# GAVLab/feature_extraction

Measured on NVIDIA B200. Metric: scans/sec, higher is better.
Workload: dtype f32

## Files before the change

feature_extraction_b200/csrc/fe_api.cu:

```cuda
#include <algorithm>
#include <cmath>
#include <cstdio>
#include <cstdlib>
#include <cstring>
#include <random>
#include <string>
#include <thread>
#include <vector>

#include "fe_kernels.cuh"

using namespace fe;

#define FE_VERSION "fe_b200 0.1 (sm_100a)"

namespace {

constexpr int GRAPH_MAX_SCANS = 16;
static_assert(GRAPH_MAX_SCANS <= 32, "k_kp_offsets_gather_small gives every scan a warp of one 1024-thread block");
struct GraphKey {
  int nscans, nch, by, k1flags, stride, xo, yo, zo;
  int desc, wantKc, bnd, epoch, lean;
  const void* pts;
  bool operator==(const GraphKey& o) const { return memcmp(this, &o, sizeof(GraphKey)) == 0; }
// ... 413 lines not shown
  CK(cudaFuncSetAttribute(k_ring_runs_wide, cudaFuncAttributeMaxDynamicSharedMemorySize, (int)(NW_RR * sizeof(RunBufT<RW2>))));
  CK(cudaFuncSetAttribute(k_cluster_rings<ECAP_L, NTL, 1, false>, cudaFuncAttributeMaxDynamicSharedMemorySize, (int)kClusterSmemL2));
  CK(cudaFuncSetAttribute(k_merge_keypoints<ECAP_M, NTM, 8, false>, cudaFuncAttributeMaxDynamicSharedMemorySize, (int)kClusterSmemM));
  CK(cudaFuncSetAttribute(k_merge_keypoints<ECAP_L, NT2, 1, false>, cudaFuncAttributeMaxDynamicSharedMemorySize, (int)kClusterSmemL));
  CK(cudaFuncSetAttribute(k_extract_clusters_stage<false>, cudaFuncAttributeMaxDynamicSharedMemorySize, (int)kClusterSmemL));
  CK(cudaFuncSetAttribute(k_desc_hist_warp, cudaFuncAttributeMaxDynamicSharedMemorySize, (int)desc_warp_smem_bytes()));
  CK(cudaFuncSetAttribute(k_desc_hist<256, DCAP, DW_CAP, false, true>, cudaFuncAttributeMaxDynamicSharedMemorySize, (int)desc_smem_bytes(DCAP, 256)));
  CK(cudaFuncSetAttribute(k_desc_hist<512, DCAP_M, DCAP, false, false>, cudaFuncAttributeMaxDynamicSharedMemorySize,
                          (int)desc_smem_bytes(DCAP_M, 512)));
  CK(cudaFuncSetAttribute(k_desc_hist<512, DCAP_L, DCAP_M, true, false>, cudaFuncAttributeMaxDynamicSharedMemorySize,
                          (int)desc_smem_bytes(DCAP_L, 512)));
  CK(cudaFuncSetAttribute(k_surface_grid_cells<NT_SURF>, cudaFuncAttributeMaxDynamicSharedMemorySize,
                          (int)surf_cells_smem_bytes(SURF_MAX_CELLS)));
  return FE_OK;
}

void launch_desc_hist(fe_ctx* ctx, Slot& s, int nscans, const DevParams& P, int gridKp, bool records, bool lean = false) {
  const int descStride = records ? FE_RECORD_FLOATS : FE_DESC_LEN, descOff = records ? 5 : 0;
#define FE_DESC_ARGS s.d_kpOut, s.d_kpScan, s.d_kpOff, nscans, s.d_kpNbr, s.d_sorted, surf_index(ctx, s), s.d_scan_off, P, \
                     s.d_rho, ctx->d_lut, ctx->d_axes, ctx->axesCap, s.d_keyA, s.d_kpNbrOff, s.d_kpRank, FE_DESC_LIST, s.d_desc, descStride, descOff, s.d_ctr, warpCap
  static const int perSm = []() {
    int v = 0;
    if (cudaOccupancyMaxActiveBlocksPerMultiprocessor(&v, k_desc_hist<256, DCAP, DW_CAP, false, true>, 256, desc_smem_bytes(DCAP, 256)) != cudaSuccess) v = 4;
    return v;
  }();
  const int warpCap = DW_CAP;
  if (nscans <= GRAPH_MAX_SCANS) {
    k_desc_hist_small<<<std::min(gridKp, ctx->numSms * 4), DW_CAP, 0, s.stream>>>(
        s.d_kpOut, s.d_kpScan, s.d_kpOff, nscans, s.d_kpNbr, s.d_sorted, s.d_scan_off, P, s.d_rho, ctx->d_lut, ctx->d_axes, ctx->axesCap,
        s.d_keyA, s.d_kpNbrOff, s.d_kpRank, s.d_desc, descStride, descOff, s.d_ctr);
    ctx->launches++;
  } else {
    static const int perSmW = []() {
      int v = 0;
      if (cudaOccupancyMaxActiveBlocksPerMultiprocessor(&v, k_desc_hist_warp, DW_WARPS * 32, desc_warp_smem_bytes()) != cudaSuccess) v = 2;
      return v;
    }();
    const int nsm = ctx->numSms;
    k_desc_hist_warp<<<nsm * std::max(perSmW, 1), DW_WARPS * 32, desc_warp_smem_bytes(), s.stream>>>(
        s.d_kpOut, s.d_kpScan, s.d_kpOff, nscans, s.d_kpNbr, s.d_sorted, s.d_scan_off, P, s.d_rho, ctx->d_lut, ctx->d_axes, ctx->axesCap,
        s.d_keyA, s.d_kpNbrOff, s.d_kpRank, s.d_desc, descStride, descOff, s.d_ctr);
    ctx->launches++;
  }
#define FE_DESC_LIST nullptr, nullptr
  k_desc_hist<256, DCAP, DW_CAP, false, true><<<std::min(gridKp, ctx->numSms * std::max(perSm, 1)), 256, desc_smem_bytes(DCAP, 256), s.stream>>>(FE_DESC_ARGS);
#undef FE_DESC_LIST
  ctx->launches++;
  if (!lean) {
#define FE_DESC_LIST s.d_kpListM, &s.d_ctr->n_list_m
  k_desc_hist<512, DCAP_M, DCAP, false, false><<<std::min(gridKp, ctx->numSms * 2), 512, desc_smem_bytes(DCAP_M, 512), s.stream>>>(FE_DESC_ARGS);
#undef FE_DESC_LIST
#define FE_DESC_LIST s.d_kpListL, &s.d_ctr->n_list_l
  k_desc_hist<512, DCAP_L, DCAP_M, true, false><<<std::min(gridKp, ctx->numSms), 512, desc_smem_bytes(DCAP_L, 512), s.stream>>>(FE_DESC_ARGS);
#undef FE_DESC_LIST
  ctx->launches += 2;
  }
#undef FE_DESC_ARGS
  if (records) {
    k_record_frame<<<ctx->numSms * 2, 256, 0, s.stream>>>(s.d_kpOut, s.d_kpOff, nscans, s.d_desc, descStride, FE_DESC_LEN);
    ctx->launches++;
  }
}

void launch_desc_mark(fe_ctx* ctx, Slot& s, int nscans, const DevParams& P, int gridKp) {
  const long long nbrCap = (long long)std::min<int64_t>(s.capPts, 0x7fffffff - MARK_LCAP);
  static const int perSm = []() {
    int v = 0;
    if (cudaOccupancyMaxActiveBlocksPerMultiprocessor(&v, k_desc_mark, 256, MARK_LCAP * sizeof(unsigned)) != cudaSuccess) v = 4;
    return v;
  }();
  gridKp = std::min(gridKp, ctx->numSms * std::max(perSm, 1));
  k_desc_mark<<<gridKp, 256, MARK_LCAP * sizeof(unsigned), s.stream>>>(s.d_kpOut, s.d_kpScan, s.d_kpOff, nscans, s.d_sorted,
                                                                       surf_index(ctx, s), s.d_scan_off, P, s.d_rho, s.d_kpNbr,
                                                                       s.d_keyA, nbrCap, s.d_kpNbrOff, s.d_ctr);
  k_kp_rank<<<(int)((s.capKp + 255) / 256), 256, 0, s.stream>>>(s.d_kpScan, s.d_kpOff, nscans, s.d_kpNbr, s.d_kpRank, s.d_kpListM, s.d_kpListL, s.d_ctr);
  ctx->launches += 2;
}

void launch_surface_grid(fe_ctx* ctx, Slot& s, int nscans, const DevParams& P, cudaStream_t q) {
  const int ncells = P.sg_nx * P.sg_ny;
  if (ncells <= SURF_MAX_CELLS) {
    k_surface_grid_cells<NT_SURF><<<nscans, NT_SURF, surf_cells_smem_bytes(ncells), q>>>(
        s.d_surf, s.d_surfCnt, s.d_scan_off, s.d_chunk_off, P, s.d_kpOut, s.d_kpOff, s.d_sorted, s.d_rho,
        s.d_surfN, s.d_ctr, s.d_ovfSurf, s.d_gridHdr, grid_hdr_bytes(ncells), s.d_tabOk);
    ctx->launches++;
    if (s.maxScanPts <= 65535 && ncells <= GRID_TAB_CAP) return;
    k_surface_grid<<<std::min(nscans, ctx->numSms * 2), NT2, 0, q>>>(s.d_surf, s.d_surfCnt, s.d_scan_off, s.d_chunk_off, P, s.d_keyA,
                                                                   s.d_keyB, s.d_valA, s.d_valB, s.d_sorted, s.d_sortedKey,
                                                                   s.d_rowStart, s.d_surfN, s.d_ctr, s.d_ovfSurf, &s.d_ctr->ovf_surf,
                                                                   s.d_tabOk, s.d_rho);
  } else {
    k_surface_grid<<<nscans, NT2, 0, q>>>(s.d_surf, s.d_surfCnt, s.d_scan_off, s.d_chunk_off, P, s.d_keyA, s.d_keyB, s.d_valA,
                                                 s.d_valB, s.d_sorted, s.d_sortedKey, s.d_rowStart, s.d_surfN, s.d_ctr, nullptr, nullptr,
                                                 s.d_tabOk, s.d_rho);
  }
  ctx->launches++;
}

int density_blocks_per_scan(int nscans, int64_t npts) {
  return (int)std::max<int64_t>(1, std::min<int64_t>(16, npts / std::max(nscans, 1) / 8192 + 1));
}

void launch_density(fe_ctx* ctx, Slot& s, int nscans, const DevParams& P, int64_t npts) {
  if (nscans <= 0) return;
  const int by = density_blocks_per_scan(nscans, npts);
  k_density<<<dim3((unsigned)nscans, (unsigned)by), 256, 0, s.stream>>>(s.d_sorted, surf_index(ctx, s), s.d_scan_off, P, s.d_surfN, s.d_rho, s.d_ctr->dens_work);
  ctx->launches++;
}

void mark(fe_ctx* ctx, Slot& s, const char* name);

void launch_clustering(fe_ctx* ctx, Slot& s, int nscans, bool singleRing, bool wantKc, bool merge, bool marks = false, bool lean = false) {
  const DevParams& P = ctx->dp;
  const int gridL = std::min(nscans, ctx->numSms), gridG = std::min(nscans, NGLOBAL);
  const size_t smemG = cluster_smem_bytes_global(NT2);
  int* ovfR = &s.d_ctr->ovf_rings;
  int* ovfR2 = &s.d_ctr->ovf_rings2;
  int* ovfM = &s.d_ctr->ovf_merge;
  int* ovfM2 = &s.d_ctr->ovf_merge2;
  float4* kc = wantKc ? s.d_kcPool : nullptr;
  int* kcB = wantKc ? s.d_kcBase : nullptr;
  int* kcC = wantKc ? s.d_kcCnt : nullptr;
  const int sr = singleRing ? 1 : 0;
#define FE_K2_ARGS s.d_crop, s.d_cropMeta, s.d_cropCnt, s.d_scan_off, s.d_chunk_off, P, sr, s.d_kfPool, s.capKf, s.d_kfBase, s.d_kfCnt, kc, \
                   s.capKc, kcB, kcC, s.d_ctr
  if (ctx->gridClustering) {
    k_cluster_rings<ECAP, NTF, 4, false><<<nscans, NTF, kClusterSmem, s.stream>>>(FE_K2_ARGS, nullptr, nullptr, s.d_ovfRings, ovfR, nullptr);
    ctx->launches++;
  } else {
#define FE_RR_ARGS s.d_crop, s.d_cropMeta, s.d_cropCnt, s.d_scan_off, s.d_chunk_off, P, sr, s.d_ringPts, s.d_ringBase, s.d_kfPool, s.capKf, \
                   s.d_kfBase, s.d_kfCnt, kc, s.capKc, kcB, kcC, s.d_ctr, s.d_ovfRuns, &s.d_ctr->ovf_runs, s.d_scanFlag, s.d_ovfRings, ovfR
    if (nscans <= GRAPH_MAX_SCANS)
      k_ring_runs<NW_RR_SMALL><<<nscans, NW_RR_SMALL * 32, sizeof(RingRunsSmT<RW, NW_RR_SMALL>), s.stream>>>(FE_RR_ARGS);
    else
      k_ring_runs<NW_RR><<<nscans, NT_RR, sizeof(RingRunsSmT<RW>), s.stream>>>(FE_RR_ARGS);
#undef FE_RR_ARGS
    ctx->launches++;
    if (!lean) {
      k_ring_runs_wide<<<std::min(nscans * 4, ctx->numSms * 7), NT_RR, NW_RR * sizeof(RunBufT<RW2>), s.stream>>>(
          s.d_scan_off, P, s.d_ringPts, s.d_ringBase, s.d_kfPool, s.capKf, s.d_kfBase, s.d_kfCnt, kc, s.capKc, kcB, kcC, s.d_ctr,
          s.d_ovfRuns, &s.d_ctr->ovf_runs, s.d_scanFlag, s.d_ovfRings, ovfR);
      ctx->launches++;
    }
  }
  if (!lean) {
    k_cluster_rings<ECAP_L, NTL, 1, false><<<gridL, NTL, kClusterSmemL2, s.stream>>>(FE_K2_ARGS, s.d_ovfRings, ovfR, s.d_ovfRings2, ovfR2, nullptr);
    k_cluster_rings<ECAP_G, NT2, 1, true><<<gridG, NT2, smemG, s.stream>>>(FE_K2_ARGS, s.d_ovfRings2, ovfR2, nullptr, nullptr, s.d_slabs);
    ctx->launches += 2;
  }
#undef FE_K2_ARGS
  if (marks) mark(ctx, s, "K2 ring clusters");
  if (merge) {
#define FE_K3_ARGS s.d_kfPool, s.d_kfBase, s.d_kfCnt, P, s.d_kpPool, (int)s.capKp, s.d_kpBase, s.d_kpCnt, s.d_ctr
    k_merge_keypoints<ECAP_M, NTM, 8, false><<<nscans, NTM, kClusterSmemM, s.stream>>>(FE_K3_ARGS, nullptr, nullptr, s.d_ovfMerge, ovfM, nullptr);
    ctx->launches++;
    if (!lean) {
      k_merge_keypoints<ECAP_L, NT2, 1, false><<<gridL, NT2, kClusterSmemL, s.stream>>>(FE_K3_ARGS, s.d_ovfMerge, ovfM, s.d_ovfMerge2, ovfM2, nullptr);
      k_merge_keypoints<ECAP_G, NT2, 1, true><<<gridG, NT2, smemG, s.stream>>>(FE_K3_ARGS, s.d_ovfMerge2, ovfM2, nullptr, nullptr, s.d_slabs);
      ctx->launches += 2;
    }
#undef FE_K3_ARGS
  }
}


BoundarySpec boundary_spec(const fe_ctx* ctx) {
  BoundarySpec B;
// ... 1193 lines not shown
```

feature_extraction_b200/csrc/fe_kernels.cuh:

```cuda
#pragma once
#include <math.h>
#include "fe_device.cuh"
#include "glibc_f32.h"
#include "sort_replay.h"
#include "../../include/fe_b200.h"

namespace fe {

constexpr int CH = 2048;
constexpr int MAXCHUNK = 512;
constexpr int NT2 = 512;
constexpr int ECAP = 1408;
constexpr int NTF = 256;
constexpr int ECAP_M = 512;
constexpr int NTM = 64;
constexpr int NTL = 1024;
constexpr int ECAP_G = 65535;
constexpr int NGLOBAL = 32;
constexpr int BRUTE_PAIRS_RINGS = 0;
constexpr int BRUTE_PAIRS_MERGE = 256;
constexpr int ECAP_L = 6144;

enum {
  ERR_RING_CAP = 1,
  ERR_KF_POOL = 2,
  ERR_KP_POOL = 4,
  ERR_MERGE_CAP = 8,
  ERR_AXIS_CAP = 16,
  ERR_CHUNKS = 32,
  ERR_KC_POOL = 64
};

enum { F_ELEV = 1, F_ROT = 2, F_CROP = 4, F_RING = 8, F_SURF = 16 };

struct DevParams {
  float xmin, xmax, ymin, ymax, zmin, zmax;
  float sx0, sx1, sy0, sy1, sz0, sz1;
  float sg_inv;
  int sg_nx, sg_ny, sg_bx;
  float tol_f, r2f_cluster;
  int min_count, max_count;
  double two_radius_threshold;
  double radius_threshold;
  float merge_tol_f, r2f_merge;
  int min_channels;
  float R2f, rho2f, Rpad, rhopad;
  float halopad;
  float zs0, zs_inv_range;
  float radii[16], theta[12], phi[13];
  int estimate_descriptors;
  int angle_libm;
};

struct DevCounters {
  int kf_cursor;
  int kp_cursor;
  int kc_cursor;
  int err;
  int kp_total;
  int ovf_rings;
  int ovf_rings2;
  int ovf_merge;
  int ovf_surf;
  int desc_unordered;
  int ovf_merge2;
  int ovf_runs;
  unsigned long long nbr_cursor;
  int kd_cursor;
  int kw_cursor;
  int n_list_m, n_list_l;
  unsigned long long dens_work[2];
};

__device__ __noinline__ float elevation_deg_literal(float xf, float yf, float zf) {
  const double x = xf, y = yf, z = zf;
  const double az = atan2(y, x);
  double sn, cs;
  sincos(az, &sn, &cs);
  const double xp = __dadd_rn(__dmul_rn(cs, x), __dmul_rn(sn, y));
  const double eld = __ddiv_rn(__dmul_rn(atan2(z, xp), 180.0), 3.14159265358979323846);
  return (float)eld;
}

__device__ __forceinline__ float elevation_deg(float xf, float yf, float zf) {
  const double x = xf, y = yf, z = zf;
  const double r2 = fma(x, x, y * y);
// ... 949 lines not shown
    const int s = scan_of_keypoint(kpOff, n_scans, g);
    kpOut[g] = kpPool[kpBase[s] + (g - kpOff[s])];
    kpScan[g] = s;
  }
}

__global__ void __launch_bounds__(1024) k_kp_offsets_gather_small(const int* __restrict__ kpCnt, int n_scans, int* __restrict__ kpOff,
                                                                   DevCounters* ctr, const float4* __restrict__ kpPool,
                                                                   const int* __restrict__ kpBase, float4* __restrict__ kpOut,
                                                                   int* __restrict__ kpScan) {
  __shared__ int sc[40];
  __shared__ int s_off[33];
  const int t = threadIdx.x, lane = t & 31, w = t >> 5;
  const int v = (t < n_scans) ? kpCnt[t] : 0;
  int tot;
  const int pos = block_excl_scan<1024>(v, &tot, sc);
  if (t < n_scans) { kpOff[t] = pos; s_off[t] = pos; }
  if (t == 0) { kpOff[n_scans] = tot; s_off[n_scans] = tot; ctr->kp_total = tot; }
  __syncthreads();
  if (w < n_scans) {
    const int o = s_off[w], n = s_off[w + 1] - o, b = kpBase[w];
    for (int i = lane; i < n; i += 32) { kpOut[o + i] = kpPool[b + i]; kpScan[o + i] = w; }
  }
}

__global__ void k_piece_counts(const int* __restrict__ cnt, const int* __restrict__ chunk_off,
                               int n_scans, int* __restrict__ perScan) {
  const int s = blockIdx.x * blockDim.x + threadIdx.x;
  if (s >= n_scans) return;
  int t = 0;
  for (int c = chunk_off[s]; c < chunk_off[s + 1]; c++) t += cnt[c];
  perScan[s] = t;
}

__global__ void __launch_bounds__(256) k_gather_chunks(
    const float4* __restrict__ src, const int* __restrict__ cnt, const long long* __restrict__ scan_off,
    const int* __restrict__ chunk_off, const int* __restrict__ outOff, float4* __restrict__ dst) {
  const int s = blockIdx.x;
  long long o = outOff[s];
  const long long base = scan_off[s];
  const int c0 = chunk_off[s], c1 = chunk_off[s + 1];
  for (int c = c0; c < c1; c++) {
    const int n = cnt[c];
    for (int j = threadIdx.x; j < n; j += blockDim.x) dst[o + j] = src[base + (long long)(c - c0) * CH + j];
    o += n;
  }
}

__global__ void __launch_bounds__(256) k_gather_pool16(
    const float4* __restrict__ pool, const int* __restrict__ pBase, const int* __restrict__ pCnt,
    const int* __restrict__ outOff, float4* __restrict__ dst) {
  const int s = blockIdx.x;
  long long o = outOff[s];
  for (int g = 0; g < 16; g++) {
    const int n = pCnt[s * 16 + g], b = pBase[s * 16 + g];
    for (int j = threadIdx.x; j < n; j += blockDim.x) dst[o + j] = pool[b + j];
    o += n;
  }
}

__global__ void __launch_bounds__(1024) k_offsets_scan(const int* __restrict__ cnt, int n, int* __restrict__ off) {
  __shared__ int sc[40];
  int run = 0;
  for (int s0 = 0; s0 < n; s0 += 1024) {
    const int s = s0 + threadIdx.x;
    const int v = (s < n) ? cnt[s] : 0;
    int tot;
    const int pos = block_excl_scan<1024>(v, &tot, sc);
    if (s < n) off[s] = run + pos;
    run += tot;
  }
  if (threadIdx.x == 0) off[n] = run;
}

__global__ void k_pool16_counts(const int* __restrict__ pCnt, int n_scans, int* __restrict__ perScan) {
  const int s = blockIdx.x * blockDim.x + threadIdx.x;
  if (s >= n_scans) return;
  int t = 0;
  for (int g = 0; g < 16; g++) t += pCnt[s * 16 + g];
  perScan[s] = t;
}

__device__ __forceinline__ int surf_cell(float v, float o, float inv, int n) {
  int c = (int)floorf((v - o) * inv);
  return max(0, min(c, n - 1));
}

struct SurfGlobalSm {
  int pre[MAXCHUNK + 1];
  int sc[40];
  unsigned wc[(NT2 / 32) * 257];
  unsigned rbase[256 + 32];
};

__device__ void surface_grid_scan_global(
    SurfGlobalSm& M, const int s, const float4* __restrict__ surf, const int* __restrict__ surfCnt,
    const long long* __restrict__ scan_off, const int* __restrict__ chunk_off, const DevParams& P,
    unsigned* __restrict__ keyA, unsigned* __restrict__ keyB, unsigned* __restrict__ valA,
    unsigned* __restrict__ valB, float4* __restrict__ sorted, unsigned* __restrict__ sortedKey,
    int* __restrict__ rowStart, int* __restrict__ surfN, DevCounters* __restrict__ ctr, int* __restrict__ rho) {
  int* pre = M.pre;
  int* sc = M.sc;
  unsigned* wc = M.wc;
  unsigned* rbase = M.rbase;
  const int tid = threadIdx.x;
  const long long base = scan_off[s];
  const int nch = chunk_off[s + 1] - chunk_off[s];
  int* rs = rowStart + (long long)s * (P.sg_ny + 1);
  if (nch > MAXCHUNK) { if (tid == 0) { atomicOr(&ctr->err, ERR_CHUNKS); surfN[s] = 0; } return; }
  const int n = chunk_prefix<NT2>(surfCnt + chunk_off[s], nch, pre, sc);
  if (tid == 0) surfN[s] = n;
  if (n == 0) {
    for (int r = tid; r <= P.sg_ny; r += NT2) rs[r] = 0;
    return;
  }
  unsigned* kA = keyA + base; unsigned* kB = keyB + base;
  unsigned* vA = valA + base; unsigned* vB = valB + base;
  for (int i = tid; i < n; i += NT2) rho[base + i] = 0;
  for (int i = tid; i < n; i += NT2) {
    const long long pp = piece_pos(pre, nch, i, base);
    const float4 q = surf[pp];
    const int cx = surf_cell(q.x, P.sx0, P.sg_inv, P.sg_nx), cy = surf_cell(q.y, P.sy0, P.sg_inv, P.sg_ny);
    kA[i] = ((unsigned)cy << P.sg_bx) | (unsigned)cx;
    vA[i] = (unsigned)(pp - base);
  }
  const int keybits = P.sg_bx + bits_for(P.sg_ny - 1);
  unsigned *kS = kA, *kT = kB, *vS = vA, *vT = vB;
  for (int shift = 0; shift < keybits; shift += 8) {
    unsigned* ki = kS; unsigned* ko = kT; unsigned* vi = vS; unsigned* vo = vT;
    block_radix_pass<NT2, unsigned>(
        n, [=](int i) { return (ki[i] >> shift) & 255u; },
        [=](int i, int pos) { ko[pos] = ki[i]; vo[pos] = vi[i]; }, wc, rbase);
    kS = ko; kT = ki; vS = vo; vT = vi;
  }
  __syncthreads();
  float4* so = sorted + base;
  unsigned* sk = sortedKey + base;
  for (int i = tid; i < n; i += NT2) {
    const unsigned k = kS[i];
    so[i] = surf[base + vS[i]];
    sk[i] = k;
    const int r = (int)(k >> P.sg_bx);
    const int rp = (i == 0) ? -1 : (int)(kS[i - 1] >> P.sg_bx);
    for (int rr = rp + 1; rr <= r; rr++) rs[rr] = i;
    if (i == n - 1) for (int rr = r + 1; rr <= P.sg_ny; rr++) rs[rr] = n;
  }
}


__global__ void __launch_bounds__(NT2, 2) k_surface_grid(
    const float4* __restrict__ surf, const int* __restrict__ surfCnt,
    const long long* __restrict__ scan_off, const int* __restrict__ chunk_off, DevParams P,
    unsigned* __restrict__ keyA, unsigned* __restrict__ keyB, unsigned* __restrict__ valA,
    unsigned* __restrict__ valB, float4* __restrict__ sorted, unsigned* __restrict__ sortedKey,
    int* __restrict__ rowStart, int* __restrict__ surfN, DevCounters* __restrict__ ctr,
    const int* __restrict__ scanList, const int* __restrict__ nList, int* __restrict__ tabOk, int* __restrict__ rho) {
  __shared__ SurfGlobalSm M;
  if (!scanList) {
    if (threadIdx.x == 0) tabOk[blockIdx.x] = 0;
    surface_grid_scan_global(M, blockIdx.x, surf, surfCnt, scan_off, chunk_off, P, keyA, keyB, valA, valB, sorted, sortedKey,
                             rowStart, surfN, ctr, rho);
  } else {
    const int n = *nList;
    for (int i = blockIdx.x; i < n; i += gridDim.x) {
      __syncthreads();
      if (threadIdx.x == 0) tabOk[scanList[i]] = 0;
      surface_grid_scan_global(M, scanList[i], surf, surfCnt, scan_off, chunk_off, P, keyA, keyB, valA, valB, sorted,
                               sortedKey, rowStart, surfN, ctr, rho);
    }
  }
}

constexpr int NT_SURF = 512;
constexpr int SURF_MAX_CELLS = 57344;

constexpr int GRID_TAB_CAP = 28672;
constexpr int GRID_MAX_SLABS = 16;
constexpr int GRID_SLAB_MIN_POINTS = 20000;
__host__ __device__ constexpr long long grid_hdr_bytes(int ncells) {
  return (long long)((ncells + 31) / 32) * 4 + (long long)((((ncells + 31) / 32) + 2) / 2) * 4 + 8 + (long long)(GRID_TAB_CAP + 2) * 2;
}
constexpr size_t surf_cells_smem_bytes(int ncells) {
  return (size_t)((GRID_TAB_CAP + 2) / 2) * 4 + 64 + (size_t)((ncells + 31) / 32) * 4 + 16 + (size_t)((ncells + 31) / 32 + 2) * 2 + 16;
}

__device__ __forceinline__ int z_slab(float z, float zs0, float zs_scale, int ns) {
  const int l = (int)floorf((z - zs0) * zs_scale);
  return max(0, min(l, ns - 1));
}

template <int NTS>
__global__ void __launch_bounds__(NTS) k_surface_grid_cells(
    const float4* __restrict__ surf, const int* __restrict__ surfCnt,
    const long long* __restrict__ scan_off, const int* __restrict__ chunk_off, DevParams P,
    const float4* __restrict__ kpOut, const int* __restrict__ kpOff,
    float4* __restrict__ sorted, int* __restrict__ rho,
    int* __restrict__ surfN, DevCounters* __restrict__ ctr, int* __restrict__ ovfList,
    unsigned char* __restrict__ gridHdr, long long gridStride, int* __restrict__ tabOk) {
  extern __shared__ __align__(16) unsigned char smem_raw[];
  const int nx = P.sg_nx, ny = P.sg_ny, ncells = nx * ny, nbm = (ncells + 31) / 32;
  unsigned* cnts = (unsigned*)smem_raw;
  unsigned* halo = cnts + ((GRID_TAB_CAP + 2) / 2) + 16;
  unsigned short* wpre = (unsigned short*)(halo + nbm + 4);
  __shared__ int sc[40];
  __shared__ int s_n, s_hc, s_hl;
  const int s = blockIdx.x, tid = threadIdx.x, lane = tid & 31, w = tid >> 5;
  constexpr int NW = NTS / 32;
  const long long base = scan_off[s];
  const int c0 = chunk_off[s];
  const int nch = chunk_off[s + 1] - c0;
  const int k0 = kpOff[s], k1 = kpOff[s + 1];
  if (tid == 0) s_hl = 0;
  if (k1 == k0) {
    if (tid == 0) { surfN[s] = 0; tabOk[s] = 1; }
    return;
  }
  {
    int v = 0;
    for (int c = tid; c < nch; c += NTS) v += surfCnt[c0 + c];
    int tot;
    block_excl_scan<NTS>(v, &tot, sc);
    if (tid == 0) s_n = tot;
  }
  for (int i = tid; i < nbm; i += NTS) halo[i] = 0u;
  __syncthreads();
  if (s_n > 65535) {
    if (tid == 0) { ovfList[atomicAdd(&ctr->ovf_surf, 1)] = s; tabOk[s] = 0; }
    return;
  }
  for (int k = k0 + w; k < k1; k += NW) {
    const float4 o = kpOut[k];
    if (!finite3(o.x, o.y, o.z)) continue;
    const int cx0 = surf_cell(o.x - P.halopad, P.sx0, P.sg_inv, nx), cx1 = surf_cell(o.x + P.halopad, P.sx0, P.sg_inv, nx);
    const int cy0 = surf_cell(o.y - P.halopad, P.sy0, P.sg_inv, ny), cy1 = surf_cell(o.y + P.halopad, P.sy0, P.sg_inv, ny);
    const int bw = cx1 - cx0 + 1, nb = bw * (cy1 - cy0 + 1);
    for (int t = lane; t < nb; t += 32) {
      const int cell = (cy0 + t / bw) * nx + cx0 + t % bw;
      atomicOr(&halo[cell >> 5], 1u << (cell & 31));
    }
  }
  __syncthreads();
  {
    int run = 0;
    for (int w0 = 0; w0 < nbm; w0 += NTS) {
      const int i = w0 + tid;
      const int v = (i < nbm) ? __popc(halo[i]) : 0;
      int tot;
      const int pos = block_excl_scan<NTS>(v, &tot, sc);
      if (i < nbm) wpre[i] = (unsigned short)(run + pos);
      run += tot;
    }
    if (tid == 0) { wpre[nbm] = (unsigned short)run; s_hc = run; }
  }
  __syncthreads();
  const int hc = s_hc;
  const int NS = (s_n >= GRID_SLAB_MIN_POINTS) ? max(1, min(GRID_MAX_SLABS, GRID_TAB_CAP / max(hc, 1))) : 1;
  if (hc > GRID_TAB_CAP) {
    if (tid == 0) { ovfList[atomicAdd(&ctr->ovf_surf, 1)] = s; tabOk[s] = 0; }
    return;
  }
  const int nslots = hc * NS, nwords = (nslots + 2) / 2;
  const float zscale = (float)NS * P.zs_inv_range;
  for (int i = tid; i < nwords; i += NTS) cnts[i] = 0u;
  __syncthreads();
  auto slot_of = [&](float x, float y, float z) -> int {
    const int cell = surf_cell(y, P.sy0, P.sg_inv, ny) * nx + surf_cell(x, P.sx0, P.sg_inv, nx);
    const unsigned bits = halo[cell >> 5];
    if (!((bits >> (cell & 31)) & 1u)) return -1;
    const int rk = (int)wpre[cell >> 5] + __popc(bits & ((1u << (cell & 31)) - 1u));
    return rk * NS + z_slab(z, P.zs0, zscale, NS);
  };
  unsigned* hlist = cnts + ((nwords + 3) & ~3);
  const int hlCap = max(0, ((GRID_TAB_CAP + 2) / 2 - ((nwords + 3) & ~3)) / 2);
  for (int it = w; it < nch * (CH / 128); it += NW) {
    const int c = it / (CH / 128);
    const int j1 = surfCnt[c0 + c];
    const float4* src = surf + base + (long long)c * CH;
    const int j = (it % (CH / 128)) * 128 + lane;
    if (j - lane >= j1) continue;
    float4 q[4];
#pragma unroll
    for (int k = 0; k < 4; k++) q[k] = (j + 32 * k < j1) ? src[j + 32 * k] : make_float4(0.f, 0.f, 0.f, 0.f);
#pragma unroll
    for (int k = 0; k < 4; k++) {
      int sl = -1;
      if (j + 32 * k < j1) sl = slot_of(q[k].x, q[k].y, q[k].z);
      if (sl >= 0) atomicAdd(&cnts[sl >> 1], (sl & 1) ? 65536u : 1u);
      const unsigned hm = __ballot_sync(FE_FULL, sl >= 0);
      if (hm) {
        int at = 0;
        if (lane == __ffs(hm) - 1) at = atomicAdd(&s_hl, __popc(hm));
        at = __shfl_sync(FE_FULL, at, __ffs(hm) - 1) + __popc(hm & lanemask_lt());
        if (sl >= 0 && at < hlCap) { hlist[2 * at] = (unsigned)(c * CH + j + 32 * k); hlist[2 * at + 1] = (unsigned)sl; }
      }
    }
  }
  __syncthreads();
  {
    const int per = (nwords + NTS - 1) / NTS;
    const int wb = min(tid * per, nwords), we = min(wb + per, nwords);
    int sum = 0;
    for (int i = wb; i < we; i++) { const unsigned v = cnts[i]; sum += (int)(v & 0xFFFFu) + (int)(v >> 16); }
    int tot;
    int run = block_excl_scan<NTS>(sum, &tot, sc);
    for (int i = wb; i < we; i++) {
      const unsigned v = cnts[i];
      const int lo = (int)(v & 0xFFFFu), hi = (int)(v >> 16);
      cnts[i] = (unsigned)run | ((unsigned)(run + lo) << 16);
      run += lo + hi;
    }
    if (tid == 0) s_n = tot;
  }
  __syncthreads();
  const int n = s_n;
  if (tid == 0) { surfN[s] = n; tabOk[s] = 1; }
  {
    unsigned* g = (unsigned*)(gridHdr + (long long)s * gridStride);
    for (int i = tid; i < nbm; i += NTS) g[i] = halo[i];
    unsigned* gp = g + nbm;
    const unsigned* wp32 = (const unsigned*)wpre;
    const int npw = (nbm + 2) / 2;
    for (int i = tid; i < npw; i += NTS) gp[i] = wp32[i];
    unsigned* gm = gp + npw;
    if (tid == 0) { gm[0] = (unsigned)NS; gm[1] = (unsigned)hc; }
    unsigned* gt = gm + 2;
    for (int i = tid; i < nwords; i += NTS) gt[i] = cnts[i];
  }
  for (int i = tid; i < n; i += NTS) rho[base + i] = 0;
  __syncthreads();
  if (n == 0) return;
  float4* so = sorted + base;
  if (s_hl <= hlCap) {
    const int nl = s_hl;
    for (int e = tid; e < nl; e += NTS) {
      const unsigned sl = hlist[2 * e + 1];
      const float4 q = surf[base + hlist[2 * e]];
      const unsigned old = atomicAdd(&cnts[sl >> 1], (sl & 1) ? 65536u : 1u);
      so[(sl & 1) ? (int)(old >> 16) : (int)(old & 0xFFFFu)] = q;
    }
    return;
  }
  for (int it = w; it < nch * (CH / 128); it += NW) {
    const int c = it / (CH / 128);
    const int j1 = surfCnt[c0 + c];
    const float4* src = surf + base + (long long)c * CH;
    const int j = (it % (CH / 128)) * 128 + lane;
    if (j - lane >= j1) continue;
    float4 q[4];
#pragma unroll
    for (int k = 0; k < 4; k++) q[k] = (j + 32 * k < j1) ? src[j + 32 * k] : make_float4(0.f, 0.f, 0.f, 0.f);
#pragma unroll
    for (int k = 0; k < 4; k++) {
      if (j + 32 * k < j1) {
        const int sl = slot_of(q[k].x, q[k].y, q[k].z);
        if (sl >= 0) {
          const unsigned old = atomicAdd(&cnts[sl >> 1], (sl & 1) ? 65536u : 1u);
          so[(sl & 1) ? (int)(old >> 16) : (int)(old & 0xFFFFu)] = q[k];
        }
      }
    }
  }
}

struct SurfIndex {
  const unsigned* sortedKey;
  const int* rowStart;
  const unsigned char* gridHdr;
  long long gridStride;
  const int* tabOk;
};

struct ScanGrid {
  const unsigned* bm;
  const unsigned short* wpre;
  const unsigned short* tab;
  int ns, hc, ncells;
  const unsigned* sk;
  const int* rs;
  int nx, bx;
  float zs0, zscale;
  __device__ __forceinline__ int rank_lb(int cell) const {
    if (cell >= ncells) return hc;
    const unsigned bits = bm[cell >> 5];
    return (int)wpre[cell >> 5] + __popc(bits & ((1u << (cell & 31)) - 1u));
  }
  __device__ __forceinline__ void row_span(int r, int cx0, int cx1, int& b, int& e) const {
    if (bm) {
      b = (int)tab[rank_lb(r * nx + cx0) * ns];
      e = (int)tab[rank_lb(r * nx + cx1 + 1) * ns];
      return;
    }
    const int rb = rs[r], re = rs[r + 1];
    const unsigned klo = ((unsigned)r << bx) | (unsigned)cx0, khi = ((unsigned)r << bx) | (unsigned)cx1;
    int lo = rb, hi = re;
    while (lo < hi) { const int mid = (lo + hi) >> 1; if (sk[mid] < klo) lo = mid + 1; else hi = mid; }
    b = lo;
    hi = re;
    while (lo < hi) { const int mid = (lo + hi) >> 1; if (sk[mid] <= khi) lo = mid + 1; else hi = mid; }
    e = lo;
  }
  __device__ __forceinline__ void cell_slabs(int cell, int l0, int l1, int& b, int& e) const {
    const unsigned bits = bm[cell >> 5];
    if (!((bits >> (cell & 31)) & 1u)) { b = e = 0; return; }
    const int rk = (int)wpre[cell >> 5] + __popc(bits & ((1u << (cell & 31)) - 1u));
    b = (int)tab[rk * ns + l0];
    e = (int)tab[rk * ns + l1 + 1];
  }
  __device__ __forceinline__ void cell_slab_span(int cell, float zlo, float zhi, int& b, int& e) const {
    const unsigned bits = bm[cell >> 5];
    if (!((bits >> (cell & 31)) & 1u)) { b = e = 0; return; }
    const int rk = (int)wpre[cell >> 5] + __popc(bits & ((1u << (cell & 31)) - 1u));
    b = (int)tab[rk * ns + z_slab(zlo, zs0, zscale, ns)];
    e = (int)tab[rk * ns + z_slab(zhi, zs0, zscale, ns) + 1];
  }
};

__device__ __forceinline__ ScanGrid scan_grid(const SurfIndex& X, int s, long long base, const DevParams& P) {
  ScanGrid G;
  G.sk = X.sortedKey + base;
  G.rs = X.rowStart + (long long)s * (P.sg_ny + 1);
  G.nx = P.sg_nx; G.bx = P.sg_bx;
  G.bm = nullptr; G.wpre = nullptr; G.tab = nullptr; G.ns = 1; G.hc = 0; G.ncells = P.sg_nx * P.sg_ny;
  G.zs0 = P.zs0; G.zscale = P.zs_inv_range;
  if (X.gridHdr && X.tabOk[s]) {
    const int nbm = (P.sg_nx * P.sg_ny + 31) / 32;
    const unsigned* g = (const unsigned*)(X.gridHdr + (long long)s * X.gridStride);
    G.bm = g;
    G.wpre = (const unsigned short*)(g + nbm);
    const unsigned* gm = g + nbm + (nbm + 2) / 2;
    G.ns = (int)gm[0];
    G.hc = (int)gm[1];
    G.tab = (const unsigned short*)(gm + 2);
    G.zscale = (float)G.ns * P.zs_inv_range;
  }
  return G;
}

constexpr int KD_BATCH = 4;
constexpr int DCAP = 1536;
constexpr int DCAP_M = 4096;
constexpr int DCAP_L = 8192;
constexpr int MARK_WCAP = 512;
constexpr int MARK_LCAP = 8 * MARK_WCAP;

__global__ void __launch_bounds__(256) k_desc_mark(
    const float4* __restrict__ kpOut, const int* __restrict__ kpScan, const int* __restrict__ kpOff,
    int n_scans, const float4* __restrict__ sorted, SurfIndex X, const long long* __restrict__ scan_off, DevParams P,
    int* __restrict__ rho, int* __restrict__ kpNbr, unsigned* __restrict__ nbrPool, long long nbrCap,
    int* __restrict__ kpNbrOff, DevCounters* __restrict__ ctr) {
  extern __shared__ __align__(16) unsigned char smem_raw[];
  unsigned* s_list = (unsigned*)smem_raw;
  __shared__ int s_wcnt[8];
  __shared__ long long s_off;
  const int total = kpOff[n_scans];
  const int lane = threadIdx.x & 31, w = threadIdx.x >> 5;
  unsigned* mylist = s_list + w * MARK_WCAP;
  for (int g = blockIdx.x; g < total; g += gridDim.x) {
    const float4 o = kpOut[g];
    const int s = kpScan[g];
    int wcnt = 0;
    if (finite3(o.x, o.y, o.z)) {
      const long long base = scan_off[s];
      const float4* so = sorted + base;
      const ScanGrid G = scan_grid(X, s, base, P);
      const int cx0 = surf_cell(o.x - P.Rpad, P.sx0, P.sg_inv, P.sg_nx), cx1 = surf_cell(o.x + P.Rpad, P.sx0, P.sg_inv, P.sg_nx);
      const int cy0 = surf_cell(o.y - P.Rpad, P.sy0, P.sg_inv, P.sg_ny), cy1 = surf_cell(o.y + P.Rpad, P.sy0, P.sg_inv, P.sg_ny);
      for (int r = cy0 + w; r <= cy1; r += 8) {
        int b, e;
        G.row_span(r, cx0, cx1, b, e);
        for (int i0 = b; i0 < e; i0 += 32) {
          const int i = i0 + lane;
          bool isn = false;
          if (i < e) {
            const float4 q = so[i];
            isn = l2_simple(o.x, o.y, o.z, q.x, q.y, q.z) < P.R2f;
            if (isn) rho[base + i] = -(s + 1);
          }
          const unsigned m = __ballot_sync(FE_FULL, isn);
          const int pos = wcnt + __popc(m & lanemask_lt());
          if (isn && pos < MARK_WCAP) mylist[pos] = (unsigned)i;
          wcnt += __popc(m);
        }
      }
    }
    if (lane == 0) s_wcnt[w] = wcnt;
    __syncthreads();
    int n = 0, before = 0;
    bool fits = true;
#pragma unroll
    for (int k = 0; k < 8; k++) {
      const int c = s_wcnt[k];
      if (k < w) before += c;
      n += c;
      fits = fits && (c <= MARK_WCAP);
    }
    if (threadIdx.x == 0) {
      kpNbr[g] = n;
      long long off = -1;
      if (n > 0 && fits) {
        off = (long long)atomicAdd(&ctr->nbr_cursor, (unsigned long long)n);
        if (off + n > nbrCap) off = -1;
      }
      s_off = off;
      kpNbrOff[g] = (int)off;
    }
    __syncthreads();
    const long long off = s_off;
    if (off >= 0)
      for (int t = lane; t < wcnt; t += 32) nbrPool[off + before + t] = mylist[t];
  }
}

__global__ void __launch_bounds__(256) k_kp_rank(const int* __restrict__ kpScan, const int* __restrict__ kpOff, int n_scans,
                                                 const int* __restrict__ kpNbr, int* __restrict__ kpRank,
                                                 int* __restrict__ listM, int* __restrict__ listL, DevCounters* __restrict__ ctr) {
  const int total = kpOff[n_scans];
  const int g = blockIdx.x * blockDim.x + threadIdx.x;
  if (g >= total) return;
  int c = 0;
  for (int j = kpOff[kpScan[g]]; j < g; j++) c += (kpNbr[j] > 0) ? 1 : 0;
  kpRank[g] = c;
  const int nb = kpNbr[g];
  if (nb > DCAP_M) listL[atomicAdd(&ctr->n_list_l, 1)] = g;
  else if (nb > DCAP) listM[atomicAdd(&ctr->n_list_m, 1)] = g;
}

constexpr int DENS_TILE = 1024;
__global__ void __launch_bounds__(256) k_density(
    const float4* __restrict__ sorted, SurfIndex X, const long long* __restrict__ scan_off, DevParams P,
    const int* __restrict__ surfN, int* __restrict__ rho, unsigned long long* __restrict__ tests) {
  __shared__ unsigned short s_list[DENS_TILE];
  __shared__ int s_wsum[8];
  const int s = blockIdx.x, tid = threadIdx.x, lane = tid & 31, w = tid >> 5;
  const int n = surfN[s];
  if (n == 0) return;
  const long long base = scan_off[s];
  const float4* so = sorted + base;
  int* rh = rho + base;
  const ScanGrid G = scan_grid(X, s, base, P);
  const int nx = P.sg_nx, ny = P.sg_ny;
  unsigned ntest = 0, nmark = 0;
  for (int t0 = (int)blockIdx.y * DENS_TILE; t0 < n; t0 += (int)gridDim.y * DENS_TILE) {
    int cntw = 0;
    unsigned mk[DENS_TILE / 256];
#pragma unroll
    for (int k = 0; k < DENS_TILE / 256; k++) {
      const int i = t0 + (w * (DENS_TILE / 256) + k) * 32 + lane;
      mk[k] = __ballot_sync(FE_FULL, i < n && rh[i] < 0);
      cntw += __popc(mk[k]);
    }
    __syncthreads();
    if (lane == 0) s_wsum[w] = cntw;
    __syncthreads();
    int off = 0, m = 0;
#pragma unroll
    for (int k = 0; k < 8; k++) { if (k < w) off += s_wsum[k]; m += s_wsum[k]; }
#pragma unroll
    for (int k = 0; k < DENS_TILE / 256; k++) {
      if ((mk[k] >> lane) & 1u) s_list[off + __popc(mk[k] & lanemask_lt())] = (unsigned short)((w * (DENS_TILE / 256) + k) * 32 + lane);
      off += __popc(mk[k]);
    }
    __syncthreads();
    for (int tw = (tid & ~31); tw < m; tw += 256) {
      const int t = tw + lane;
      const bool act = t < m;
      const int i = t0 + (int)s_list[act ? t : tw];
      const float4 p = so[i];
      const int cx0 = surf_cell(p.x - P.rhopad, P.sx0, P.sg_inv, nx), cx1 = surf_cell(p.x + P.rhopad, P.sx0, P.sg_inv, nx);
      const int cy0 = surf_cell(p.y - P.rhopad, P.sy0, P.sg_inv, ny), cy1 = surf_cell(p.y + P.rhopad, P.sy0, P.sg_inv, ny);
      int cnt = 0;
      if (G.bm && G.ns > 1) {
        const float zlo = p.z - P.rhopad, zhi = p.z + P.rhopad;
        const int ux0 = __reduce_min_sync(FE_FULL, cx0), ux1 = __reduce_max_sync(FE_FULL, cx1);
        const int uy0 = __reduce_min_sync(FE_FULL, cy0), uy1 = __reduce_max_sync(FE_FULL, cy1);
        if ((ux1 - ux0 + 1) * (uy1 - uy0 + 1) <= 16) {
          const int l0 = __reduce_min_sync(FE_FULL, z_slab(zlo, G.zs0, G.zscale, G.ns));
          const int l1 = __reduce_max_sync(FE_FULL, z_slab(zhi, G.zs0, G.zscale, G.ns));
          for (int r = uy0; r <= uy1; r++)
            for (int c = ux0; c <= ux1; c++) {
              int b, e;
              G.cell_slabs(r * nx + c, l0, l1, b, e);
              for (int j = b; j < e; j++) {
                const float4 q = so[j];
                if (l2_simple(p.x, p.y, p.z, q.x, q.y, q.z) < P.rho2f) cnt++;
              }
              if (act) ntest += (unsigned)(e - b);
            }
        } else {
          for (int r = cy0; r <= cy1; r++)
            for (int c = cx0; c <= cx1; c++) {
              int b, e;
              G.cell_slab_span(r * nx + c, zlo, zhi, b, e);
              for (int j = b; j < e; j++) {
                const float4 q = so[j];
                if (l2_simple(p.x, p.y, p.z, q.x, q.y, q.z) < P.rho2f) cnt++;
              }
              if (act) ntest += (unsigned)(e - b);
            }
        }
      } else {
        for (int r = cy0; r <= cy1; r++) {
          int b, e;
          G.row_span(r, cx0, cx1, b, e);
          for (int j = b; j < e; j++) {
            const float4 q = so[j];
            if (l2_simple(p.x, p.y, p.z, q.x, q.y, q.z) < P.rho2f) cnt++;
          }
          if (act) ntest += (unsigned)(e - b);
        }
      }
      if (!act) continue;
      rh[i] = cnt;
      nmark++;
    }
  }
  if (tests) {
    unsigned long long a = ntest, b = nmark;
#pragma unroll
    for (int d = 16; d; d >>= 1) { a += __shfl_xor_sync(FE_FULL, a, d); b += __shfl_xor_sync(FE_FULL, b, d); }
    if (lane == 0 && b) { atomicAdd(&tests[0], a); atomicAdd(&tests[1], b); }
  }
}

__device__ __forceinline__ float eigen_sum3(float a0, float a1, float a2) {
  return __fadd_rn(a0, __fadd_rn(a1, a2));
}

constexpr size_t desc_smem_bytes(int cap, int nt) {
  return (size_t)cap * 24 + FE_DESC_LEN * 4 + 64 + 0 * nt;
}

__device__ __forceinline__ bool shape_context_contribution(const float4 o, const float4 q, const float d2, const float axx,
                                                           const float axy, const DevParams& P, const float* __restrict__ lut,
                                                           const int dens, int& bin, float& wgt) {
  if (fabsf(d2 - 0.0f) < 1.17549435e-38f) return false;
  if (dens <= 0) return false;
  const float axz = -0.0f;
  const float rr = __fsqrt_rn(d2);
  const float pox = __fsub_rn(q.x, o.x), poy = __fsub_rn(q.y, o.y), poz = __fsub_rn(q.z, o.z);
  const float lambda = eigen_sum3(__fmul_rn(0.0f, pox), __fmul_rn(0.0f, poy), __fmul_rn(1.0f, poz));
  float prx = __fsub_rn(__fsub_rn(q.x, __fmul_rn(lambda, 0.0f)), o.x);
  float pry = __fsub_rn(__fsub_rn(q.y, __fmul_rn(lambda, 0.0f)), o.y);
  float prz = __fsub_rn(__fsub_rn(q.z, __fmul_rn(lambda, 1.0f)), o.z);
  {
    const float inv = __fdiv_rn(1.0f, __fsqrt_rn(eigen_sum3(__fmul_rn(prx, prx), __fmul_rn(pry, pry), __fmul_rn(prz, prz))));
    prx = __fmul_rn(prx, inv); pry = __fmul_rn(pry, inv); prz = __fmul_rn(prz, inv);
  }
  const float crx = __fsub_rn(__fmul_rn(axy, prz), __fmul_rn(axz, pry));
  const float cry = __fsub_rn(__fmul_rn(axz, prx), __fmul_rn(axx, prz));
  const float crz = __fsub_rn(__fmul_rn(axx, pry), __fmul_rn(axy, prx));
  const float crn = __fsqrt_rn(eigen_sum3(__fmul_rn(crx, crx), __fmul_rn(cry, cry), __fmul_rn(crz, crz)));
  const float dt = eigen_sum3(__fmul_rn(axx, prx), __fmul_rn(axy, pry), __fmul_rn(axz, prz));
  float phi = P.angle_libm ? (float)atan2((double)crn, (double)dt) : glibc::atan2f_fdlibm(crn, dt);
  phi = __fmul_rn(phi, 57.29578f);
  const float cdn = eigen_sum3(__fmul_rn(crx, 0.0f), __fmul_rn(cry, 0.0f), __fmul_rn(crz, 1.0f));
  phi = (cdn < 0.f) ? __fsub_rn(360.0f, phi) : phi;
  float nox = pox, noy = poy, noz = poz;
  {
    const float inv = __fdiv_rn(1.0f, __fsqrt_rn(eigen_sum3(__fmul_rn(nox, nox), __fmul_rn(noy, noy), __fmul_rn(noz, noz))));
    nox = __fmul_rn(nox, inv); noy = __fmul_rn(noy, inv); noz = __fmul_rn(noz, inv);
  }
  float th = eigen_sum3(__fmul_rn(0.0f, nox), __fmul_rn(0.0f, noy), __fmul_rn(1.0f, noz));
  const float t1 = (-1.0f < th) ? th : -1.0f;
  const float t2 = (t1 < 1.0f) ? t1 : 1.0f;
  th = __fmul_rn(P.angle_libm ? (float)acos((double)t2) : glibc::acosf_fdlibm(t2), 57.29578f);
  int j = 0, k = 0, l = 0;
#pragma unroll
  for (int a = 15; a >= 1; a--) if (rr <= P.radii[a]) j = a - 1;
#pragma unroll
  for (int a = 11; a >= 1; a--) if (th <= P.theta[a]) k = a - 1;
#pragma unroll
  for (int a = 12; a >= 1; a--) if (phi <= P.phi[a]) l = a - 1;
  bin = l * 165 + k * 15 + j;
  wgt = __fmul_rn(__fdiv_rn(1.0f, (float)dens), lut[bin]);
  return true;
}

template <int NT, int CAP, int NB_MIN, bool LAST, bool DYN>
__global__ void __launch_bounds__(NT) k_desc_hist(
    const float4* __restrict__ kpOut, const int* __restrict__ kpScan, const int* __restrict__ kpOff,
    int n_scans, const int* __restrict__ kpNbr, const float4* __restrict__ sorted, SurfIndex X,
    const long long* __restrict__ scan_off, DevParams P, const int* __restrict__ rho,
    const float* __restrict__ lut, const float2* __restrict__ axes, int axesCap,
    const unsigned* __restrict__ nbrPool, const int* __restrict__ kpNbrOff, const int* __restrict__ kpRank,
    const int* __restrict__ glist, const int* __restrict__ nlist, float* __restrict__ desc, int descStride, int descOff,
    DevCounters* __restrict__ ctr, int warpCap) {
// ... 663 lines not shown
```

Measured before the change: 2.927 million.

## Narrow density neighbor search with circular row windows and x-subcell grid tables

When z-slabs are not used, the per-scan grid table now splits each cell into x sub-cells, and a flag bit marks this in the header. The density kernel clips each grid row to the chord of the search circle at that row's y-gap, then looks up a tight start and end at sub-cell resolution. This is meant to cut the number of candidate points tested against the radius. The first three rows are also merged into one flattened loop to reduce divergence, and k_density gets a min-blocks launch bound. The cost is extra table entries and per-row window maths, with conservative slack terms to keep the results exact.

New measurement: 2.758 million (median of 6 runs). 0.942x the previous value.

```diff
diff --git a/feature_extraction_b200/csrc/fe_api.cu b/feature_extraction_b200/csrc/fe_api.cu
--- a/feature_extraction_b200/csrc/fe_api.cu
+++ b/feature_extraction_b200/csrc/fe_api.cu
@@ -519,7 +519,8 @@
   if (ncells <= SURF_MAX_CELLS) {
     k_surface_grid_cells<NT_SURF><<<nscans, NT_SURF, surf_cells_smem_bytes(ncells), q>>>(
         s.d_surf, s.d_surfCnt, s.d_scan_off, s.d_chunk_off, P, s.d_kpOut, s.d_kpOff, s.d_sorted, s.d_rho,
-        s.d_surfN, s.d_ctr, s.d_ovfSurf, s.d_gridHdr, grid_hdr_bytes(ncells), s.d_tabOk);
+        s.d_surfN, s.d_ctr, s.d_ovfSurf, s.d_gridHdr, grid_hdr_bytes(ncells), s.d_tabOk,
+        nscans <= GRAPH_MAX_SCANS ? 1 : GRID_NX_MAX);
     ctx->launches++;
     if (s.maxScanPts <= 65535 && ncells <= GRID_TAB_CAP) return;
     k_surface_grid<<<std::min(nscans, ctx->numSms * 2), NT2, 0, q>>>(s.d_surf, s.d_surfCnt, s.d_scan_off, s.d_chunk_off, P, s.d_keyA,
diff --git a/feature_extraction_b200/csrc/fe_kernels.cuh b/feature_extraction_b200/csrc/fe_kernels.cuh
--- a/feature_extraction_b200/csrc/fe_kernels.cuh
+++ b/feature_extraction_b200/csrc/fe_kernels.cuh
@@ -2,6 +2,7 @@
 #include <math.h>
 #include "fe_device.cuh"
 #include "glibc_f32.h"
+#include "surf_window.h"
 #include "sort_replay.h"
 #include "../../include/fe_b200.h"
 
@@ -1117,8 +1118,7 @@
 }
 
 __device__ __forceinline__ int surf_cell(float v, float o, float inv, int n) {
-  int c = (int)floorf((v - o) * inv);
-  return max(0, min(c, n - 1));
+  return sw::t_cell(sw::grid_t(v, o, inv), n);
 }
 
 struct SurfGlobalSm {
@@ -1211,6 +1211,8 @@
 
 constexpr int GRID_TAB_CAP = 28672;
 constexpr int GRID_MAX_SLABS = 16;
+constexpr int GRID_NX_MAX = 4;
+constexpr unsigned GRID_XSUB = 1u << 16;
 constexpr int GRID_SLAB_MIN_POINTS = 20000;
 __host__ __device__ constexpr long long grid_hdr_bytes(int ncells) {
   return (long long)((ncells + 31) / 32) * 4 + (long long)((((ncells + 31) / 32) + 2) / 2) * 4 + 8 + (long long)(GRID_TAB_CAP + 2) * 2;
@@ -1231,7 +1233,7 @@
     const float4* __restrict__ kpOut, const int* __restrict__ kpOff,
     float4* __restrict__ sorted, int* __restrict__ rho,
     int* __restrict__ surfN, DevCounters* __restrict__ ctr, int* __restrict__ ovfList,
-    unsigned char* __restrict__ gridHdr, long long gridStride, int* __restrict__ tabOk) {
+    unsigned char* __restrict__ gridHdr, long long gridStride, int* __restrict__ tabOk, int nxMax) {
   extern __shared__ __align__(16) unsigned char smem_raw[];
   const int nx = P.sg_nx, ny = P.sg_ny, ncells = nx * ny, nbm = (ncells + 31) / 32;
   unsigned* cnts = (unsigned*)smem_raw;
@@ -1289,7 +1291,9 @@
   }
   __syncthreads();
   const int hc = s_hc;
-  const int NS = (s_n >= GRID_SLAB_MIN_POINTS) ? max(1, min(GRID_MAX_SLABS, GRID_TAB_CAP / max(hc, 1))) : 1;
+  const bool slabs = s_n >= GRID_SLAB_MIN_POINTS;
+  const int fit = max(1, GRID_TAB_CAP / max(hc, 1));
+  const int NS = slabs ? min(GRID_MAX_SLABS, fit) : (1 << (31 - __clz(min(nxMax, fit))));
   if (hc > GRID_TAB_CAP) {
     if (tid == 0) { ovfList[atomicAdd(&ctr->ovf_surf, 1)] = s; tabOk[s] = 0; }
     return;
@@ -1299,11 +1303,13 @@
   for (int i = tid; i < nwords; i += NTS) cnts[i] = 0u;
   __syncthreads();
   auto slot_of = [&](float x, float y, float z) -> int {
-    const int cell = surf_cell(y, P.sy0, P.sg_inv, ny) * nx + surf_cell(x, P.sx0, P.sg_inv, nx);
+    const float tx = sw::grid_t(x, P.sx0, P.sg_inv);
+    const int cx = sw::t_cell(tx, nx);
+    const int cell = surf_cell(y, P.sy0, P.sg_inv, ny) * nx + cx;
     const unsigned bits = halo[cell >> 5];
     if (!((bits >> (cell & 31)) & 1u)) return -1;
     const int rk = (int)wpre[cell >> 5] + __popc(bits & ((1u << (cell & 31)) - 1u));
-    return rk * NS + z_slab(z, P.zs0, zscale, NS);
+    return rk * NS + (slabs ? z_slab(z, P.zs0, zscale, NS) : sw::t_sub(tx, cx, NS));
   };
   unsigned* hlist = cnts + ((nwords + 3) & ~3);
   const int hlCap = max(0, ((GRID_TAB_CAP + 2) / 2 - ((nwords + 3) & ~3)) / 2);
@@ -1357,7 +1363,7 @@
     const int npw = (nbm + 2) / 2;
     for (int i = tid; i < npw; i += NTS) gp[i] = wp32[i];
     unsigned* gm = gp + npw;
-    if (tid == 0) { gm[0] = (unsigned)NS; gm[1] = (unsigned)hc; }
+    if (tid == 0) { gm[0] = (unsigned)NS | (slabs ? 0u : GRID_XSUB); gm[1] = (unsigned)hc; }
     unsigned* gt = gm + 2;
     for (int i = tid; i < nwords; i += NTS) gt[i] = cnts[i];
   }
@@ -1410,9 +1416,10 @@
   const unsigned short* wpre;
   const unsigned short* tab;
   int ns, hc, ncells;
+  int xsub;
   const unsigned* sk;
   const int* rs;
-  int nx, bx;
+  int nx, ny, bx;
   float zs0, zscale;
   __device__ __forceinline__ int rank_lb(int cell) const {
     if (cell >= ncells) return hc;
@@ -1434,6 +1441,17 @@
     while (lo < hi) { const int mid = (lo + hi) >> 1; if (sk[mid] <= khi) lo = mid + 1; else hi = mid; }
     e = lo;
   }
+  __device__ __forceinline__ void row_window(int r, float tpx, float tpy, float padt, int& b, int& e) const {
+    int ca, sa, cb, sb;
+    sw::row_window(tpx, tpy, padt, r, nx, ny, xsub ? ns : 1, ca, sa, cb, sb);
+    if (!bm) { row_span(r, ca, cb, b, e); return; }
+    const int cA = r * nx + ca, cB = r * nx + cb;
+    const unsigned bA = bm[cA >> 5], bB = bm[cB >> 5];
+    const int rA = (int)wpre[cA >> 5] + __popc(bA & ((1u << (cA & 31)) - 1u));
+    const int rB = (int)wpre[cB >> 5] + __popc(bB & ((1u << (cB & 31)) - 1u));
+    b = (int)tab[rA * ns + (((bA >> (cA & 31)) & 1u) ? sa : 0)];
+    e = (int)tab[rB * ns + (((bB >> (cB & 31)) & 1u) ? (xsub ? sb + 1 : ns) : 0)];
+  }
   __device__ __forceinline__ void cell_slabs(int cell, int l0, int l1, int& b, int& e) const {
     const unsigned bits = bm[cell >> 5];
     if (!((bits >> (cell & 31)) & 1u)) { b = e = 0; return; }
@@ -1454,8 +1472,8 @@
   ScanGrid G;
   G.sk = X.sortedKey + base;
   G.rs = X.rowStart + (long long)s * (P.sg_ny + 1);
-  G.nx = P.sg_nx; G.bx = P.sg_bx;
-  G.bm = nullptr; G.wpre = nullptr; G.tab = nullptr; G.ns = 1; G.hc = 0; G.ncells = P.sg_nx * P.sg_ny;
+  G.nx = P.sg_nx; G.ny = P.sg_ny; G.bx = P.sg_bx;
+  G.bm = nullptr; G.wpre = nullptr; G.tab = nullptr; G.ns = 1; G.xsub = 0; G.hc = 0; G.ncells = P.sg_nx * P.sg_ny;
   G.zs0 = P.zs0; G.zscale = P.zs_inv_range;
   if (X.gridHdr && X.tabOk[s]) {
     const int nbm = (P.sg_nx * P.sg_ny + 31) / 32;
@@ -1463,7 +1481,8 @@
     G.bm = g;
     G.wpre = (const unsigned short*)(g + nbm);
     const unsigned* gm = g + nbm + (nbm + 2) / 2;
-    G.ns = (int)gm[0];
+    G.ns = (int)(gm[0] & (GRID_XSUB - 1u));
+    G.xsub = (gm[0] & GRID_XSUB) ? 1 : 0;
     G.hc = (int)gm[1];
     G.tab = (const unsigned short*)(gm + 2);
     G.zscale = (float)G.ns * P.zs_inv_range;
@@ -1561,7 +1580,7 @@
 }
 
 constexpr int DENS_TILE = 1024;
-__global__ void __launch_bounds__(256) k_density(
+__global__ void __launch_bounds__(256, 4) k_density(
     const float4* __restrict__ sorted, SurfIndex X, const long long* __restrict__ scan_off, DevParams P,
     const int* __restrict__ surfN, int* __restrict__ rho, unsigned long long* __restrict__ tests) {
   __shared__ unsigned short s_list[DENS_TILE];
@@ -1601,10 +1620,10 @@
       const bool act = t < m;
       const int i = t0 + (int)s_list[act ? t : tw];
       const float4 p = so[i];
-      const int cx0 = surf_cell(p.x - P.rhopad, P.sx0, P.sg_inv, nx), cx1 = surf_cell(p.x + P.rhopad, P.sx0, P.sg_inv, nx);
       const int cy0 = surf_cell(p.y - P.rhopad, P.sy0, P.sg_inv, ny), cy1 = surf_cell(p.y + P.rhopad, P.sy0, P.sg_inv, ny);
       int cnt = 0;
-      if (G.bm && G.ns > 1) {
+      if (G.bm && !G.xsub && G.ns > 1) {
+        const int cx0 = surf_cell(p.x - P.rhopad, P.sx0, P.sg_inv, nx), cx1 = surf_cell(p.x + P.rhopad, P.sx0, P.sg_inv, nx);
         const float zlo = p.z - P.rhopad, zhi = p.z + P.rhopad;
         const int ux0 = __reduce_min_sync(FE_FULL, cx0), ux1 = __reduce_max_sync(FE_FULL, cx1);
         const int uy0 = __reduce_min_sync(FE_FULL, cy0), uy1 = __reduce_max_sync(FE_FULL, cy1);
@@ -1634,9 +1653,22 @@
             }
         }
       } else {
-        for (int r = cy0; r <= cy1; r++) {
+        const float tx = sw::grid_t(p.x, P.sx0, P.sg_inv), ty = sw::grid_t(p.y, P.sy0, P.sg_inv);
+        const float padt = __fmul_rn(P.rhopad, P.sg_inv);
+        int b0, e0, b1 = 0, e1 = 0, b2 = 0, e2 = 0;
+        G.row_window(cy0, tx, ty, padt, b0, e0);
+        if (cy0 + 1 <= cy1) G.row_window(cy0 + 1, tx, ty, padt, b1, e1);
+        if (cy0 + 2 <= cy1) G.row_window(cy0 + 2, tx, ty, padt, b2, e2);
+        const int n0 = e0 - b0, n01 = n0 + (e1 - b1), nt = n01 + (e2 - b2);
+        const int o1 = b1 - n0, o2 = b2 - n01;
+        for (int k = 0; k < nt; k++) {
+          const float4 q = so[k + (k < n0 ? b0 : (k < n01 ? o1 : o2))];
+          if (l2_simple(p.x, p.y, p.z, q.x, q.y, q.z) < P.rho2f) cnt++;
+        }
+        if (act) ntest += (unsigned)nt;
+        for (int r = cy0 + 3; r <= cy1; r++) {
           int b, e;
-          G.row_span(r, cx0, cx1, b, e);
+          G.row_window(r, tx, ty, padt, b, e);
           for (int j = b; j < e; j++) {
             const float4 q = so[j];
             if (l2_simple(p.x, p.y, p.z, q.x, q.y, q.z) < P.rho2f) cnt++;
diff --git a/feature_extraction_b200/csrc/surf_window.h b/feature_extraction_b200/csrc/surf_window.h
--- /dev/null
+++ b/feature_extraction_b200/csrc/surf_window.h
@@ -0,0 +1,45 @@
+#pragma once
+#include <math.h>
+
+#include "glibc_f32.h"
+
+namespace fe {
+namespace sw {
+
+constexpr float SLACK = 9.5367431640625e-07f;
+
+FE_HD float grid_t(float v, float origin, float inv) { return glibc::f_mul(glibc::f_sub(v, origin), inv); }
+
+FE_HD int t_cell(float t, int n) {
+  const int c = (int)floorf(t);
+  return c < 0 ? 0 : (c > n - 1 ? n - 1 : c);
+}
+
+FE_HD int t_sub(float t, int c, int nsub) {
+  const int s = (int)floorf(glibc::f_mul(glibc::f_sub(t, (float)c), (float)nsub));
+  return s < 0 ? 0 : (s > nsub - 1 ? nsub - 1 : s);
+}
+
+FE_HD float gap(float tp, int k, int n) {
+  float g = 0.0f;
+  if (k < n - 1 && tp >= (float)(k + 1)) g = glibc::f_sub(tp, (float)(k + 1));
+  else if (k > 0 && tp < (float)k) g = glibc::f_sub((float)k, tp);
+  g = glibc::f_sub(g, glibc::f_mul(glibc::f_add(fabsf(tp), (float)(k + 2)), SLACK));
+  return g > 0.0f ? g : 0.0f;
+}
+
+FE_HD void row_window(float tpx, float tpy, float padt, int r, int nx, int ny, int nsub, int& ca, int& sa, int& cb,
+                      int& sb) {
+  const float gy = gap(tpy, r, ny);
+  const float h2 = glibc::f_sub(glibc::f_mul(padt, padt), glibc::f_mul(gy, gy));
+  float w = h2 > 0.0f ? glibc::f_sqrt(h2) : 0.0f;
+  w = glibc::f_add(glibc::f_mul(w, 1.0f + SLACK), glibc::f_mul(glibc::f_add(glibc::f_add(fabsf(tpx), padt), 2.0f), 8.0f * SLACK));
+  const float xa = glibc::f_sub(tpx, w), xb = glibc::f_add(tpx, w);
+  ca = t_cell(xa, nx);
+  sa = t_sub(xa, ca, nsub);
+  cb = t_cell(xb, nx);
+  sb = t_sub(xb, cb, nsub);
+}
+
+}
+}
```
